# facebookresearch/actionmesh

Hardware: AMD Instinct MI355X
Metric: denoise-steps/sec (16f x 4096tok) (higher is better)
Workload: dtype bf16; 1 GPU; headline: Stage-I denoise step, B=2 (CFG) x T=16 frames x N=4096 tokens, width 1024 (8 heads x 128), 21 layers all inflated, S=257 ctx tokens, random-init weights, seeded N(0,1) latents/context resident in HBM; parallelism=single GPU

## Files before the change

### actionmesh_amd/_lib.py

```python
from __future__ import annotations

import ctypes as C
import os
from typing import Optional

_HERE = os.path.dirname(os.path.abspath(__file__))
LIB_PATH = os.environ.get("ACTIONMESH_AMD_LIB") or os.path.join(_HERE, "libactionmesh_amd.so")
LIB_PATH_F16 = os.environ.get("ACTIONMESH_AMD_LIB_F16") or os.path.join(_HERE, "libactionmesh_amd_f16.so")
ABI_VERSION = 2


class HipLibraryMissing(RuntimeError):
    pass


class AmConfig(C.Structure):
    _fields_ = [
        ("in_channels", C.c_int32), ("num_layers", C.c_int32), ("num_heads", C.c_int32),
        ("width", C.c_int32), ("ff_inner", C.c_int32), ("cross_dim", C.c_int32),
        ("inflated_mask_lo", C.c_uint32), ("inflated_mask_hi", C.c_uint32),
        ("max_batch", C.c_int32), ("max_frames_local", C.c_int32), ("max_tokens", C.c_int32),
        ("max_ctx_tokens", C.c_int32), ("world_size", C.c_int32), ("rank", C.c_int32),
        ("attn_defer_log2", C.c_int32), ("attn_fp8", C.c_int32), ("reserved", C.c_int32 * 6),
    ]


GEMM_ACT_MASK, GEMM_ACT_GELU = 0xff, 1
GEMM_FORCE_128, GEMM_LOCKSTEP, GEMM_FORCE_256 = 0x100, 0x200, 0x400
GEMM_ABLATE_STORE, GEMM_ABLATE_READ, GEMM_ABLATE_MASK = 0x800, 0x1000, 0x1800
GEMM_SKEW_SHIFT, GEMM_SKEW_MASK = 13, 0xe000
GEMM_NO_GELU_TABLE = 0x10000


class AmGemmArgs(C.Structure):
    _fields_ = [
        ("A1", C.c_void_p), ("lda1", C.c_int32), ("K1", C.c_int32),
        ("A2", C.c_void_p), ("lda2", C.c_int32),
        ("W", C.c_void_p), ("ldw", C.c_int32),
        ("bias", C.c_void_p), ("residual", C.c_void_p),
        ("C", C.c_void_p), ("ldc", C.c_int32),
        ("M", C.c_int32), ("N", C.c_int32), ("K", C.c_int32), ("act", C.c_int32),
        ("a_G", C.c_int32), ("a_gs", C.c_int32), ("a_off", C.c_int32),
        ("c_G", C.c_int32), ("c_gs", C.c_int32), ("c_off", C.c_int32),
        ("ln_stats", C.c_void_p), ("ln_colsum", C.c_void_p), ("ln_part", C.c_void_p),
    ]


class AmHeadPostArgs(C.Structure):
    _fields_ = [
        ("X", C.c_void_p), ("ldx", C.c_int32),
        ("rows", C.c_int64), ("seq_len", C.c_int32), ("rows_per_frame", C.c_int32),
        ("heads", C.c_int32), ("nparts", C.c_int32), ("kinds", C.c_int32 * 3),
        ("w_q", C.c_void_p), ("w_k", C.c_void_p), ("eps", C.c_float),
        ("rope_cos", C.c_void_p), ("rope_sin", C.c_void_p),
        ("out_q", C.c_void_p), ("sq_pad", C.c_int32),
        ("out_k", C.c_void_p), ("out_vt", C.c_void_p), ("sk_pad", C.c_int32),
    ]


class AmNnArgs(C.Structure):
    _fields_ = [
        ("points", C.c_void_p), ("n_points", C.c_int64), ("points_bstride", C.c_int64),
        ("queries", C.c_void_p), ("n_queries", C.c_int64), ("queries_bstride", C.c_int64),
        ("batch", C.c_int32), ("precise", C.c_int32),
# ... 316 lines not shown
    "am_image_resample_workspace_bytes": (C.c_size_t, [C.c_int, C.c_int, C.c_int]),
    "am_image_resample": (C.c_int, [C.POINTER(AmImageResampleArgs), _P]),
    "am_image_materialize": (C.c_int, [C.POINTER(AmImageMaterializeArgs), _P]),
    "am_mask_refine_workspace_bytes": (C.c_size_t, [C.c_int, C.c_int, C.c_int]),
    "am_mask_refine": (C.c_int, [C.POINTER(AmMaskRefineArgs), _P]),
    "am_graph_components_workspace_bytes": (C.c_size_t, [C.c_int64, C.c_int64]),
    "am_graph_components": (C.c_int, [C.POINTER(AmGraphArgs), _P]),
    "am_vertex_normals_workspace_bytes": (C.c_size_t, [C.c_int, C.c_int64]),
    "am_vertex_normals": (C.c_int, [C.POINTER(AmVertexNormalsArgs), _P]),
    "am_face_areas": (C.c_int, [C.POINTER(AmFaceAreasArgs), _P]),
    "am_surface_sample": (C.c_int, [C.POINTER(AmSurfaceSampleArgs), _P]),
    "am_decimate_quadrics": (C.c_int, [C.POINTER(AmDecimateQuadricsArgs), _P]),
    "am_decimate_edges": (C.c_int, [C.POINTER(AmDecimateEdgesArgs), _P]),
    "am_decimate_select": (C.c_int, [C.POINTER(AmDecimateSelectArgs), _P]),
    "am_decimate_apply": (C.c_int, [C.POINTER(AmDecimateApplyArgs), _P]),
    "am_iso_classify": (C.c_int, [C.POINTER(AmIsoClassifyArgs), _P]),
    "am_iso_vertices": (C.c_int, [C.POINTER(AmIsoVerticesArgs), _P]),
    "am_iso_triangles": (C.c_int, [C.POINTER(AmIsoTrianglesArgs), _P]),
    "am_dmc_cells": (C.c_int, [C.POINTER(AmDmcCellsArgs), _P]),
    "am_dmc_classify": (C.c_int, [C.POINTER(AmDmcClassifyArgs), _P]),
    "am_dmc_vertices": (C.c_int, [C.POINTER(AmDmcVerticesArgs), _P]),
    "am_dmc_triangles": (C.c_int, [C.POINTER(AmDmcTrianglesArgs), _P]),
    "am_layer_pre_attn": (C.c_int, [_P, C.c_int, _P]),
    "am_layer_attn_local": (C.c_int, [_P, C.c_int, _P]),
    "am_layer_post_attn": (C.c_int, [_P, C.c_int, _P]),
    "am_forward_end": (C.c_int, [_P, _P, _P]),
    "am_kv_chunk_elems": (C.c_int, [_P, C.POINTER(C.c_size_t)]),
    "am_bind_kv_buffers": (C.c_int, [_P, _P, _P, C.c_size_t]),
    "am_bind_kv8_buffers": (C.c_int, [_P, _P, _P, C.c_size_t]),
    "am_attention_counters": (C.c_int, [_P, _P]),
    "am_flow_step": (C.c_int, [_P, _P, C.c_int, _P, C.c_float, C.c_int, _P, C.c_int, C.c_int, C.c_int, _P]),
    "am_step_flops": (C.c_double, [_P, C.c_int, C.c_int, C.c_int, C.c_int]),
    "am_gemm_bf16": (C.c_int, [C.POINTER(AmGemmArgs), _P]),
    "am_layernorm_bf16": (C.c_int, [_P, _P, _P, _P, C.c_int64, C.c_int, C.c_float, _P]),
    "am_add_layernorm_f32": (C.c_int, [_P, _P, _P, _P, _P, C.c_int64, C.c_int, C.c_float, _P]),
    "am_row_stats_bf16": (C.c_int, [_P, _P, C.c_int64, C.c_int, C.c_float, _P]),
    "am_row_stats_finalize": (C.c_int, [_P, C.c_int, C.c_int, _P, C.c_int64, C.c_float, _P]),
    "am_layernorm_stats_bf16": (C.c_int, [_P, _P, _P, _P, C.c_int64, C.c_int, C.c_float, _P, _P]),
    "am_ln_fold_weight": (C.c_int, [_P, _P, _P, _P, _P, _P, _P, C.c_int, C.c_int, _P]),
    "am_head_post": (C.c_int, [C.POINTER(AmHeadPostArgs), _P]),
    "am_gemm_headpost_bf16": (C.c_int, [C.POINTER(AmGemmArgs), C.POINTER(AmHeadPostArgs), _P]),
    "am_attention_bf16": (C.c_int, [C.POINTER(AmAttnArgs), _P]),
    "am_attention_quantize_fp8": (C.c_int, [C.POINTER(AmAttnArgs), _P, _P, _P, _P]),
    "am_attention_fp8": (C.c_int, [C.POINTER(AmAttnArgs), _P, _P, _P, _P]),
    "am_peer_alloc": (C.c_int, [C.c_size_t, C.POINTER(_P)]),
    "am_peer_alloc_flags": (C.c_int, [C.c_size_t, C.POINTER(_P), C.POINTER(C.c_int)]),
    "am_peer_free": (C.c_int, [_P]),
    "am_peer_export": (C.c_int, [_P, _P]),
    "am_peer_open": (C.c_int, [_P, C.POINTER(_P)]),
    "am_peer_close": (C.c_int, [_P]),
    "am_peer_copy": (C.c_int, [_P, _P, C.c_size_t, _P]),
    "am_peer_signal": (C.c_int, [_P, C.c_uint32, _P]),
    "am_peer_wait": (C.c_int, [_P, C.c_uint32, _P, _P]),
    "am_debug_trace_begin": (C.c_int, [_P, C.c_int]),
    "am_debug_trace_end": (C.c_int, [_P, C.c_int, C.POINTER(C.c_int)]),
    "am_debug_trace_stage_name": (C.c_char_p, [C.c_int]),
    "am_f32_to_bf16": (C.c_int, [_P, _P, C.c_size_t, _P]),
    "am_bf16_to_f32": (C.c_int, [_P, _P, C.c_size_t, _P]),
    "am_timestep_sinusoid": (C.c_int, [_P, _P, C.c_int, C.c_int, _P]),
    "am_forward_sharded_peer": (C.c_int, [_P, _P, _P, C.c_int, C.c_int, C.c_int, _P, C.POINTER(AmPeerRing), _P, C.c_int, _P]),
    "am_peer_ring_destroy": (C.c_int, [C.POINTER(AmPeerRing)]),
}

_libs = {}


# ... 52 lines not shown
```

### actionmesh_amd/csrc/am_gemm.hip

```cpp
#include <stdlib.h>
#include <string.h>

#include "am_common.h"

namespace {

constexpr int BM = 128, BN = 128, BK = 64;
constexpr int LDS_ROW = BK + 8;
constexpr int TILE_ELEMS = BM * LDS_ROW;
constexpr int CS_LD = BN + 4;
constexpr int SMEM_MAIN = 2 * 2 * TILE_ELEMS * (int)sizeof(bf16_t);
constexpr int SMEM_EPI = BM * CS_LD * (int)sizeof(float);
constexpr int SMEM_BYTES = SMEM_MAIN > SMEM_EPI ? SMEM_MAIN : SMEM_EPI;
constexpr int GROUP_M = 8;
constexpr int B2 = 256;

__device__ inline int64_t map_row(int r, int G, int gs, int off) {
  if (G <= 0) return r;
  int g = r / G;
  return (int64_t)g * gs + off + (r - g * G);
}

__global__ __launch_bounds__(256, 2) void gemm_bf16_kernel(am_gemm_args p, int tiles_m, int tiles_n, int m_base) {
  extern __shared__ __attribute__((aligned(16))) unsigned char smem[];
  bf16_t* As = reinterpret_cast<bf16_t*>(smem);
  bf16_t* Bs = As + 2 * TILE_ELEMS;
  float* Cs = reinterpret_cast<float*>(smem);

  const int nb = tiles_m * tiles_n;
  const int bid = blockIdx.x;
  int lid;
  {
    const int xcd = bid & 7, idx = bid >> 3;
    const int q = nb >> 3, r = nb & 7;
    lid = (xcd < r ? xcd * (q + 1) : r * (q + 1) + (xcd - r) * q) + idx;
  }
  int tm, tn;
  {
    const int group_sz = GROUP_M * tiles_n;
    const int g = lid / group_sz;
    const int first_m = g * GROUP_M;
    const int gm = min(GROUP_M, tiles_m - first_m);
    const int in_g = lid - g * group_sz;
    tm = first_m + in_g % gm;
    tn = in_g / gm;
  }
  const int m0 = m_base + tm * BM, n0 = tn * BN;
// ... 642 lines not shown
constexpr int GT_ENTRIES = 2 * (int)GT_SPAN;
constexpr int GT_BYTES = GT_ENTRIES * 2;
__global__ void gelu_table_kernel(uint16_t* tab) {
  const int i = blockIdx.x * blockDim.x + threadIdx.x;
  if (i >= GT_ENTRIES) return;
  const uint32_t sgn = (uint32_t)i / GT_SPAN, rel = (uint32_t)i - sgn * GT_SPAN;
  const bf16_t b = (bf16_t)((sgn << 15) | (rel + GT_LO));
  tab[i] = (uint16_t)(pack_bf2(gelu_erf(bf2f(b)), 0.f) & 0xffffu);
}
__device__ __forceinline__ uint32_t gelu_table_pair(uint32_t pk, const unsigned char* tab, uint32_t& bad) {
  const uint32_t b0 = pk & 0xffffu, b1 = pk >> 16;
  const uint32_t r0 = (b0 & 0x7fffu) - GT_LO, r1 = (b1 & 0x7fffu) - GT_LO;
  bad |= (uint32_t)(r0 >= GT_SPAN) | (uint32_t)(r1 >= GT_SPAN);
  const uint32_t i0 = min(r0, GT_SPAN - 1) + (b0 >> 15) * GT_SPAN, i1 = min(r1, GT_SPAN - 1) + (b1 >> 15) * GT_SPAN;
  const uint32_t g0 = *reinterpret_cast<const uint16_t*>(tab + 2u * i0);
  const uint32_t g1 = *reinterpret_cast<const uint16_t*>(tab + 2u * i1);
  return g0 | (g1 << 16);
}
__device__ __forceinline__ bool gelu_table_has(float x) {
  const uint32_t b = pack_bf2(x, 0.f) & 0x7fffu;
  return b - GT_LO < GT_SPAN;
}

constexpr int HT_BYTES = 128 * BK * 2;
constexpr int PBUF_BYTES = 4 * HT_BYTES;
constexpr int FOLD_OFF = 2 * PBUF_BYTES;
constexpr int SMEM2PP_BYTES = FOLD_OFF + 4096;
constexpr int GT_OFF = SMEM2PP_BYTES;
constexpr int SMEM2PP_GELU_BYTES = GT_OFF + GT_BYTES;

#define PP_BARRIER() do { __builtin_amdgcn_sched_barrier(0); asm volatile("s_barrier" ::: "memory"); __builtin_amdgcn_sched_barrier(0); } while (0)
#define PP_LGKM0() asm volatile("s_waitcnt lgkmcnt(0)" ::: "memory")

template <bool HP>
__global__ __launch_bounds__(512, 2) void gemm256pp_bf16_kernel(am_gemm_args p, int tiles_m, int tiles_n, int m_base, am_headpost_args hp,
                                                                 const uint16_t* gelu_tab) {
  extern __shared__ __attribute__((aligned(16))) unsigned char smem[];

  const int nb = tiles_m * tiles_n;
  const int bid = blockIdx.x;
  {
    const int units = (p.act & AM_GEMM_SKEW_MASK) >> AM_GEMM_SKEW_SHIFT;
    if (units && units < 7 && bid < 256) {
      const unsigned long long t0 = wall_clock64();
      const unsigned long long wait = (unsigned long long)(bid & 7) * units * 150ull;
      while (wall_clock64() - t0 < wait) __builtin_amdgcn_s_sleep(4);
    }
  }
  int lid;
  {
    const int xcd = bid & 7, idx = bid >> 3;
    const int q = nb >> 3, r = nb & 7;
    lid = (xcd < r ? xcd * (q + 1) : r * (q + 1) + (xcd - r) * q) + idx;
  }
  int tm, tn;
  {
    const int group_sz = GROUP_M * tiles_n;
    const int g = lid / group_sz;
    const int first_m = g * GROUP_M;
    const int gm = min(GROUP_M, tiles_m - first_m);
    const int in_g = lid - g * group_sz;
    tm = first_m + in_g % gm;
    tn = in_g / gm;
  }
  const int m0 = m_base + tm * B2, n0 = tn * B2;

  const int tid = threadIdx.x;
  const int lane = tid & 63;
  const int wave = __builtin_amdgcn_readfirstlane(tid >> 6);
  const int wm = wave >> 2, wn = wave & 3;

  const int l15 = lane & 15, l4 = lane >> 4;
  f32x4_t acc[8][4];
  {
    f32x4_t bv[4];
#pragma unroll
    for (int ni = 0; ni < 4; ++ni) {
      bv[ni] = f32x4_t{0.f, 0.f, 0.f, 0.f};
      if (p.bias && !p.ln_stats) bv[ni] = *reinterpret_cast<const f32x4_t*>(p.bias + min(n0 + wn * 64 + ni * 16 + l4 * 4, p.N - 4));
    }
#pragma unroll
    for (int ni = 0; ni < 4; ++ni) asm volatile("" : "+v"(bv[ni]));
#pragma unroll
    for (int ni = 0; ni < 4; ++ni)
#pragma unroll
      for (int mi = 0; mi < 8; ++mi) acc[mi][ni] = bv[ni];
  }
  __builtin_amdgcn_sched_barrier(0);
  if (p.ln_stats) {
    {
      const int dw = wave * 64 + lane;
      const int row = min(m0 + (dw >> 1), p.M - 1);
      __builtin_amdgcn_global_load_lds((gbl_ptr_t)(p.ln_stats + 2 * (int64_t)row + (dw & 1)), (lds_ptr_t)(smem + FOLD_OFF + wave * 256), 4, 0, 0);
    }
    {
      const int idx = (wave & 3) * 64 + lane;
      const int n = min(n0 + idx, p.N - 1);
      const float* src = wave < 4 ? p.ln_colsum + n : (p.bias ? p.bias + n : p.ln_colsum + n);
      __builtin_amdgcn_global_load_lds((gbl_ptr_t)src, (lds_ptr_t)(smem + FOLD_OFF + 2048 + wave * 256), 4, 0, 0);
    }
  }

  if (gelu_tab != nullptr) {
#pragma unroll
    for (int i = 0; i < GT_BYTES / 4 / 512; ++i)
      __builtin_amdgcn_global_load_lds((gbl_ptr_t)(reinterpret_cast<const uint32_t*>(gelu_tab) + i * 512 + wave * 64 + lane),
                                       (lds_ptr_t)(smem + GT_OFF + (i * 512 + wave * 64) * 4), 4, 0, 0);
  }

  uint32_t offA1[4], offA2[4], offW[4];
#pragma unroll
  for (int i = 0; i < 4; ++i) {
    const int half = i >> 1, pc = i & 1;
    const int r = pc * 64 + wave * 8 + (lane >> 3);
    const int c = (lane & 7) ^ ((r >> 1) & 7);
    const int ar = min(m0 + half * 128 + r, p.M - 1);
    const int64_t pr = map_row(ar, p.a_G, p.a_gs, p.a_off);
    offA1[i] = (uint32_t)(pr * (p.lda1 >> 3) + c);
    offA2[i] = (uint32_t)(pr * (p.lda2 >> 3) + c);
    const int wr = min(n0 + half * 128 + r, p.N - 1);
    offW[i] = (uint32_t)((int64_t)wr * (p.ldw >> 3) + c);
  }
  auto stage_a = [&](int half, int kt, int buf_off) __attribute__((always_inline)) {
    const int k0 = kt * BK;
    const bool first = k0 < p.K1;
    const unsigned char* base = reinterpret_cast<const unsigned char*>(first ? p.A1 + k0 : p.A2 + (k0 - p.K1));
#pragma unroll
    for (int pc = 0; pc < 2; ++pc) {
      const uint32_t off = first ? offA1[half * 2 + pc] : offA2[half * 2 + pc];
      __builtin_amdgcn_global_load_lds((gbl_ptr_t)(base + ((uint64_t)off << 4)),
                                       (lds_ptr_t)(smem + buf_off + half * HT_BYTES + (pc * 512 + wave * 64) * 16), 16, 0, 0);
    }
  };
  auto stage_w = [&](int half, int kt, int buf_off) __attribute__((always_inline)) {
    const unsigned char* base = reinterpret_cast<const unsigned char*>(p.W + kt * BK);
#pragma unroll
// ... 46 lines not shown
  PP_BARRIER();
  if (wm == 1) PP_BARRIER();

  for (int t = 0; t < nk; ++t) {
    const int cur = (t & 1) * PBUF_BYTES, nxt = PBUF_BYTES - cur;
    const int ta = min(t + 1, nk - 1), tb = min(t + 2, nk - 1);
    read_a(cur, 0); read_w(cur, 0);
    stage_a(0, ta, nxt);
    PP_LGKM0(); PP_BARRIER();
    PP_QUADRANT(0, 0);
    PP_BARRIER();
    read_w(cur, 1);
    stage_a(1, ta, nxt);
    PP_LGKM0(); PP_BARRIER();
    PP_QUADRANT(0, 1);
    PP_BARRIER();
    read_a(cur, 1);
    stage_w(0, tb, cur);
    PP_LGKM0(); PP_BARRIER();
    PP_QUADRANT(1, 1);
    PP_BARRIER();
    stage_w(1, tb, cur);
    asm volatile("s_waitcnt vmcnt(4)" ::: "memory");
    PP_BARRIER();
    PP_QUADRANT(1, 0);
    PP_BARRIER();
  }
  if (wm == 0) PP_BARRIER();
  asm volatile("s_waitcnt vmcnt(0)" ::: "memory");
  PP_BARRIER();

  ResidualPrefetch pre;
  pre.on = false;
  if constexpr (!HP) residual_prefetch(p, tid, m0, n0, pre);
  if (p.ln_stats) {
    f32x4_t cs[4], dv[4];
    const float* fold = reinterpret_cast<const float*>(smem + FOLD_OFF);
#pragma unroll
    for (int ni = 0; ni < 4; ++ni) {
      const int nl = wn * 64 + ni * 16 + l4 * 4;
      cs[ni] = *reinterpret_cast<const f32x4_t*>(fold + 512 + nl);
      dv[ni] = p.bias ? *reinterpret_cast<const f32x4_t*>(fold + 768 + nl) : f32x4_t{0.f, 0.f, 0.f, 0.f};
    }
#pragma unroll
    for (int mi = 0; mi < 8; ++mi) {
      const f32x2_t st = *reinterpret_cast<const f32x2_t*>(fold + 2 * (wm * 128 + mi * 16 + l15));
      const float nm = -st[0] * st[1];
#pragma unroll
      for (int ni = 0; ni < 4; ++ni)
#pragma unroll
        for (int e = 0; e < 4; ++e) acc[mi][ni][e] = fmaf(acc[mi][ni][e], st[1], fmaf(nm, cs[ni][e], dv[ni][e]));
    }
  }
  unsigned char* stage = smem;
  uint32_t gelu_bad = 0;
  auto stage_pass = [&](auto&& convert) __attribute__((always_inline)) {
#pragma unroll
    for (int mi = 0; mi < 8; ++mi)
#pragma unroll
      for (int ni = 0; ni < 4; ++ni) {
        const int ml = wm * 128 + mi * 16 + l15;
        const int nl = wn * 64 + ni * 16 + l4 * 4;
        const u32x2_t w = convert(acc[mi][ni]);
        const int u = (nl >> 2) ^ (ml & 15);
        *reinterpret_cast<u32x2_t*>(stage + ml * 512 + u * 8) = w;
      }
// ... 3 lines not shown
      return u32x2_t{gelu_table_pair(pack_bf2(a[0], a[1]), smem + GT_OFF, gelu_bad), gelu_table_pair(pack_bf2(a[2], a[3]), smem + GT_OFF, gelu_bad)};
    });
  } else if ((p.act & AM_GEMM_ACT_MASK) == AM_GEMM_ACT_GELU) {
    stage_pass([&](const f32x4_t& a) __attribute__((always_inline)) {
      float v[4];
#pragma unroll
      for (int e = 0; e < 4; ++e) v[e] = gelu_erf(rbf(a[e]));
      return u32x2_t{pack_bf2(v[0], v[1]), pack_bf2(v[2], v[3])};
    });
  } else {
    stage_pass([&](const f32x4_t& a) __attribute__((always_inline)) { return u32x2_t{pack_bf2(a[0], a[1]), pack_bf2(a[2], a[3])}; });
  }
  if (gelu_bad) {
#pragma unroll
    for (int mi = 0; mi < 8; ++mi)
#pragma unroll
      for (int ni = 0; ni < 4; ++ni) {
        const int ml = wm * 128 + mi * 16 + l15;
        const int nl = wn * 64 + ni * 16 + l4 * 4;
        bool any = false;
#pragma unroll
        for (int e = 0; e < 4; ++e) any |= !gelu_table_has(acc[mi][ni][e]);
        if (any) {
          uint16_t* q = reinterpret_cast<uint16_t*>(stage + ml * 512 + ((nl >> 2) ^ (ml & 15)) * 8);
#pragma unroll
          for (int e = 0; e < 4; ++e)
            if (!gelu_table_has(acc[mi][ni][e])) q[e] = (uint16_t)(pack_bf2(gelu_erf(rbf(acc[mi][ni][e])), 0.f) & 0xffffu);
        }
      }
  }
  __syncthreads();
  if constexpr (HP) store_staged_tile_headpost(p, hp, stage, tid, m0, n0);
  else store_staged_tile(p, stage, tid, m0, n0, &pre);
}
#undef PP_QUADRANT

}

static int gemm_skew_units(int rounds) {
  static int enabled[64];
  int dev = 0;
  if (hipGetDevice(&dev) != hipSuccess || dev < 0 || dev >= 64) return 0;
  if (enabled[dev] == 0) {
    hipDeviceProp_t pr;
    bool on = hipGetDeviceProperties(&pr, dev) == hipSuccess && pr.multiProcessorCount == 256 && strncmp(pr.gcnArchName, "gfx950", 6) == 0;
    const char* e = getenv("ACTIONMESH_AMD_GEMM_SKEW");
    if (e && e[0] == '0') on = false;
    enabled[dev] = on ? 1 : 2;
  }
  if (enabled[dev] != 1) return 0;
  return rounds >= 24 ? 4 : rounds >= 16 ? 3 : rounds >= 12 ? 2 : rounds >= 4 ? 1 : 0;
}

static const uint16_t* gelu_table(hipStream_t st) {
#ifdef AM_F16
  return nullptr;
#else
  static uint16_t* tab[64];
  static int state[64];
  static std::mutex mu;
  int dev = 0, cur = 0;
  if (hipGetDevice(&cur) != hipSuccess) return nullptr;
  dev = cur;
  if (st != nullptr && hipStreamGetDevice(st, &dev) != hipSuccess) { (void)hipGetLastError(); dev = cur; }
  if (dev < 0 || dev >= 64) return nullptr;
  std::lock_guard<std::mutex> lk(mu);
  if (state[dev] == 0) {
    const char* e = getenv("ACTIONMESH_AMD_GELU_TABLE");
    if (e && e[0] == '0') { state[dev] = 2; return nullptr; }
    hipStreamCaptureStatus cs = hipStreamCaptureStatusNone;
    if (hipStreamIsCapturing(st, &cs) != hipSuccess || cs != hipStreamCaptureStatusNone) { (void)hipGetLastError(); return nullptr; }
    if (dev != cur && hipSetDevice(dev) != hipSuccess) { (void)hipGetLastError(); return nullptr; }
    uint16_t* t = nullptr;
    bool ok = hipMalloc(reinterpret_cast<void**>(&t), GT_BYTES) == hipSuccess;
    if (ok) {
      hipLaunchKernelGGL(gelu_table_kernel, dim3(ceil_div(GT_ENTRIES, 256)), dim3(256), 0, st, t);
      ok = hipGetLastError() == hipSuccess && hipStreamSynchronize(st) == hipSuccess;
      if (!ok) (void)hipFree(t);
    }
    if (dev != cur) (void)hipSetDevice(cur);
    if (!ok) { (void)hipGetLastError(); return nullptr; }
    tab[dev] = t;
    state[dev] = 1;
  }
// ... 15 lines not shown
  }
}

extern "C" int am_gemm_bf16(const am_gemm_args* a, void* stream) {
  AM_CHECK(a != nullptr, "am_gemm_bf16: null args");
  AM_CHECK(a->M > 0 && a->N > 0 && a->K > 0, "am_gemm_bf16: empty problem M=%d N=%d K=%d", a->M, a->N, a->K);
  AM_CHECK(a->K % BK == 0, "am_gemm_bf16: K=%d must be a multiple of %d", a->K, BK);
  AM_CHECK(a->N % 8 == 0, "am_gemm_bf16: N=%d must be a multiple of 8", a->N);
  AM_CHECK(a->A1 && a->W && a->C, "am_gemm_bf16: null operand");
  AM_CHECK(a->K1 > 0 && a->K1 <= a->K && a->K1 % BK == 0, "am_gemm_bf16: K1=%d invalid for K=%d", a->K1, a->K);
  AM_CHECK(a->K1 == a->K || a->A2 != nullptr, "am_gemm_bf16: K1 < K requires A2");
  AM_CHECK(a->lda1 % 8 == 0 && a->ldw % 8 == 0 && a->ldc % 8 == 0 && (a->A2 == nullptr || a->lda2 % 8 == 0),
           "am_gemm_bf16: leading dimensions must be multiples of 8 elements (16 B)");
  AM_CHECK(((uintptr_t)a->A1 | (uintptr_t)a->W | (uintptr_t)a->C | (uintptr_t)a->A2 | (uintptr_t)a->residual) % 16 == 0,
           "am_gemm_bf16: operands must be 16-byte aligned");
  if (a->ln_stats) {
    AM_CHECK(a->ln_colsum != nullptr, "am_gemm_bf16: ln_stats without ln_colsum");
    AM_CHECK(a->A2 == nullptr, "am_gemm_bf16: a folded LayerNorm needs one A operand");
    AM_CHECK(a->a_G == 0 || (a->act & AM_GEMM_FORCE_128) || (a->N < 256 && !(a->act & AM_GEMM_FORCE_256)),
             "am_gemm_bf16: a folded LayerNorm over a row-mapped A needs the 128x128 kernel (N < 256 without the forced 256x256 tile)");
    AM_CHECK(!(a->act & AM_GEMM_LOCKSTEP), "am_gemm_bf16: the round-1 lockstep kernel has no folded-LayerNorm epilogue");
    AM_CHECK(((uintptr_t)a->ln_stats % 8 == 0) && ((uintptr_t)a->ln_colsum % 16 == 0) && (a->bias == nullptr || (uintptr_t)a->bias % 16 == 0) &&
             a->N % 4 == 0, "am_gemm_bf16: ln_stats / ln_colsum / bias misaligned");
  }
  if (a->ln_part) {
    AM_CHECK(a->c_G == 0, "am_gemm_bf16: ln_part needs the identity C row map");
    AM_CHECK((uintptr_t)a->ln_part % 8 == 0, "am_gemm_bf16: ln_part misaligned");
  }
  AM_ONCE_PER_DEVICE({
    AM_HIP(hipFuncSetAttribute(reinterpret_cast<const void*>(gemm_bf16_kernel),
                               hipFuncAttributeMaxDynamicSharedMemorySize, SMEM_BYTES));
    AM_HIP(hipFuncSetAttribute(reinterpret_cast<const void*>(gemm256_bf16_kernel),
                               hipFuncAttributeMaxDynamicSharedMemorySize, SMEM2_BYTES));
    AM_HIP(hipFuncSetAttribute(reinterpret_cast<const void*>(gemm256pp_bf16_kernel<false>),
                               hipFuncAttributeMaxDynamicSharedMemorySize, SMEM2PP_GELU_BYTES));
    AM_HIP(hipFuncSetAttribute(reinterpret_cast<const void*>(gemm256pp_bf16_kernel<true>),
                               hipFuncAttributeMaxDynamicSharedMemorySize, SMEM2PP_BYTES));
  });
  am_gemm_args args = *a;
  const bool force_small = (args.act & AM_GEMM_FORCE_128) != 0;
  const bool legacy = (args.act & AM_GEMM_LOCKSTEP) != 0;
  const bool force_big = (args.act & AM_GEMM_FORCE_256) != 0;
  const int abl = args.act & (AM_GEMM_ABLATE_MASK | AM_GEMM_SKEW_MASK);
  const bool no_gelu_table = (args.act & AM_GEMM_NO_GELU_TABLE) != 0;
  args.act &= AM_GEMM_ACT_MASK;
  AM_CHECK(args.act == 0 || args.act == AM_GEMM_ACT_GELU, "am_gemm_bf16: unknown activation %d", args.act);
  const bool big = !force_small && args.N >= 8 && args.M >= 1 &&
                   (force_big || (args.N >= 256 && args.M >= 1024 && (int64_t)ceil_div(args.M, B2) * ceil_div(args.N, B2) >= 192));
  AM_CHECK(!big || (uintptr_t)args.bias % 16 == 0, "am_gemm_bf16: the 256x256 tile needs a 16-byte aligned bias");
  args.act |= abl;
  float* const ln_part = args.ln_part;
  int64_t part_done = 0;
  args.ln_part = nullptr;
  if (big && (abl & AM_GEMM_SKEW_MASK) == 0) {
    const int rounds = (int)(((int64_t)ceil_div(args.M, B2) * ceil_div(args.N, B2)) / 256);
    args.act |= gemm_skew_units(rounds) << AM_GEMM_SKEW_SHIFT;
  }
  if (big) {
    const int rem = args.M % B2;
    const int m_main = (rem != 0 && rem <= 128 && args.M > 8 * B2) ? args.M - rem : args.M;
    const int tiles_m = ceil_div(m_main, B2), tiles_n = ceil_div(args.N, B2);
    if (legacy) {
      hipLaunchKernelGGL(gemm256_bf16_kernel, dim3(tiles_m * tiles_n), dim3(512), SMEM2_BYTES,
                         (hipStream_t)stream, args, tiles_m, tiles_n, 0);
    } else {
      am_gemm_args main_args = args;
      if (ln_part && args.N % B2 == 0 && !(args.act & AM_GEMM_ABLATE_MASK)) {
        main_args.ln_part = ln_part;
        part_done = (int64_t)(args.M / B2) * B2;
        if (part_done > m_main) part_done = m_main;
      }
      const uint16_t* gt = ((main_args.act & AM_GEMM_ACT_MASK) == AM_GEMM_ACT_GELU && !no_gelu_table) ? gelu_table((hipStream_t)stream) : nullptr;
      hipLaunchKernelGGL(gemm256pp_bf16_kernel<false>, dim3(tiles_m * tiles_n), dim3(512), gt ? SMEM2PP_GELU_BYTES : SMEM2PP_BYTES,
                         (hipStream_t)stream, main_args, tiles_m, tiles_n, 0, am_headpost_args{}, gt);
    }
    if (m_main < args.M) launch_tail(args, m_main, (hipStream_t)stream);
  } else {
    const int tiles_m = ceil_div(args.M, BM), tiles_n = ceil_div(args.N, BN);
    hipLaunchKernelGGL(gemm_bf16_kernel, dim3(tiles_m * tiles_n), dim3(256), SMEM_BYTES,
                       (hipStream_t)stream, args, tiles_m, tiles_n, 0);
  }
  AM_HIP(hipGetLastError());
  if (ln_part && part_done < args.M)
    AM_TRY(am_row_part(args.C, args.ldc, part_done, args.M - part_done, args.N, ln_part, stream));
  return AM_OK;
}

int am_head_post_partial(const am_headpost_args* a, int s_min_last, int s_min_other, void* stream);

extern "C" int am_gemm_headpost_bf16(const am_gemm_args* g, const am_headpost_args* hp, void* stream) {
  AM_CHECK(g && hp, "am_gemm_headpost_bf16: null argument");
  AM_CHECK(g->C == hp->X && g->ldc == hp->ldx && (int64_t)g->M == hp->rows && g->N == hp->heads * hp->nparts * 128,
           "am_gemm_headpost_bf16: the GEMM's output (C, ldc, M, N) must be the head split's input (X, ldx, rows, heads * nparts * 128)");
  bool has_v = false;
  for (int i = 0; i < hp->nparts; ++i) has_v |= hp->kinds[i] == 2;
  const int rem = g->M % B2;
  const bool tail_split = rem != 0 && rem <= 128 && g->M > 8 * B2;
  AM_CHECK(g->ln_part == nullptr, "am_gemm_headpost_bf16: no row statistics of a head-split output");
  const bool fuse = (g->act & AM_GEMM_ACT_MASK) == 0 && !g->residual && (!g->bias || g->ln_stats) && !g->A2 && g->a_G == 0 && g->c_G == 0 && g->N % 256 == 0 && g->M % 16 == 0 &&
                    g->N >= 256 && g->M >= 1024 && (int64_t)ceil_div(g->M, B2) * ceil_div(g->N, B2) >= 192 &&
                    (!has_v || hp->seq_len % 16 == 0) && (!tail_split || rem <= hp->seq_len) && hp->rows % hp->seq_len == 0 &&
                    !(g->act & (AM_GEMM_FORCE_128 | AM_GEMM_LOCKSTEP | AM_GEMM_FORCE_256)) && getenv("ACTIONMESH_AMD_NO_FUSED_QKV") == nullptr;
  if (!fuse) {
    AM_TRY(am_gemm_bf16(g, stream));
    return am_head_post(hp, stream);
  }
  AM_CHECK(g->K % BK == 0 && g->K1 == g->K && g->lda1 % 8 == 0 && g->ldw % 8 == 0, "am_gemm_headpost_bf16: bad GEMM operands");
  AM_CHECK(((uintptr_t)g->A1 | (uintptr_t)g->W | (uintptr_t)g->C) % 16 == 0, "am_gemm_headpost_bf16: operands must be 16-byte aligned");
  if (g->ln_stats)
    AM_CHECK(g->ln_colsum && (uintptr_t)g->ln_stats % 8 == 0 && (uintptr_t)g->ln_colsum % 16 == 0 && (g->bias == nullptr || (uintptr_t)g->bias % 16 == 0),
             "am_gemm_headpost_bf16: ln_stats / ln_colsum / bias missing or misaligned");
  AM_TRY(am_head_post_check(hp));
  AM_ONCE_PER_DEVICE({
    AM_HIP(hipFuncSetAttribute(reinterpret_cast<const void*>(gemm256pp_bf16_kernel<true>), hipFuncAttributeMaxDynamicSharedMemorySize, SMEM2PP_BYTES));
    AM_HIP(hipFuncSetAttribute(reinterpret_cast<const void*>(gemm_bf16_kernel), hipFuncAttributeMaxDynamicSharedMemorySize, SMEM_BYTES));
  });
  am_gemm_args args = *g;
  args.act = g->act & AM_GEMM_ABLATE_MASK;
  const int m_main = tail_split ? args.M - rem : args.M;
  const int tiles_m = ceil_div(m_main, B2), tiles_n = ceil_div(args.N, B2);
  {
    const int rounds = (int)(((int64_t)tiles_m * tiles_n) / 256);
    args.act |= gemm_skew_units(rounds) << AM_GEMM_SKEW_SHIFT;
  }
  am_gemm_args main_args = args;
  main_args.M = m_main;
  hipLaunchKernelGGL(gemm256pp_bf16_kernel<true>, dim3(tiles_m * tiles_n), dim3(512), SMEM2PP_BYTES, (hipStream_t)stream, main_args, tiles_m,
                     tiles_n, 0, *hp, (const uint16_t*)nullptr);
  if (m_main < args.M) launch_tail(args, m_main, (hipStream_t)stream);
  AM_HIP(hipGetLastError());
  const int s_min_last = hp->seq_len - (args.M - m_main);
  return am_head_post_partial(hp, s_min_last, hp->seq_len, stream);
}
```

### actionmesh_amd/ops.py

```python
from __future__ import annotations

import ctypes as C
from typing import Optional, Sequence, Tuple

import torch

from . import _lib as L
from .mesh_topology import MeshTopology

HEAD_DIM = 128


H16 = (torch.bfloat16, torch.float16)


def _entry(key, name: str):
    if isinstance(key, torch.Tensor):
        key = key.dtype
    l = L.lib(key if isinstance(key, str) else "f16" if key == torch.float16 else "bf16")
    return l, getattr(l, name)


def _call(t: torch.Tensor, key, name: str, *args) -> None:
    l, fn = _entry(key, name)
# ... 26 lines not shown


def _need_rows(t: torch.Tensor, dtype, name: str) -> torch.Tensor:
    _on_device(t, dtype, name)
    if t.dim() != 2 or t.stride(1) != 1:
        raise ValueError(f"{name}: expected a 2-D tensor with unit column stride, got shape {tuple(t.shape)} strides {t.stride()}")
    return t


def round_up(x: int, m: int) -> int:
    return (x + m - 1) // m * m


def _out_rows(out: Optional[torch.Tensor], rows: int, ld_out: int, dtype, device, name: str) -> torch.Tensor:
    if out is None:
        return torch.empty((rows, ld_out), dtype=dtype, device=device)
    _need(out, dtype, f"{name}: out")
    if tuple(out.shape) != (rows, ld_out):
        raise ValueError(f"{name}: out {tuple(out.shape)} != ({rows}, {ld_out})")
    return out


def perm16_index(n: int, device=None) -> torch.Tensor:
    k = torch.arange(n, device=device)
    return (k & ~0xC) | ((k & 4) << 1) | ((k & 8) >> 1)


def _fold_args(g, bias: Optional[torch.Tensor], ln: Optional[Tuple[torch.Tensor, torch.Tensor]]) -> None:
    if bias is not None:
        g.bias = _need(bias, torch.float32, "bias").data_ptr()
    if ln is not None:
        g.ln_stats = _need(ln[0], torch.float32, "ln stats").data_ptr()
        g.ln_colsum = _need(ln[1], torch.float32, "ln colsum").data_ptr()


def gemm(a: torch.Tensor, w: torch.Tensor, bias: Optional[torch.Tensor] = None,
         residual: Optional[torch.Tensor] = None, gelu: bool = False,
         a2: Optional[torch.Tensor] = None, out: Optional[torch.Tensor] = None,
         a_map: Tuple[int, int, int] = (0, 0, 0), c_map: Tuple[int, int, int] = (0, 0, 0),
         M: Optional[int] = None, force_small: bool = False, legacy: bool = False,
         force_big: bool = False, ablate: int = 0,
         ln: Optional[Tuple[torch.Tensor, torch.Tensor]] = None, ln_part: Optional[torch.Tensor] = None,
         gelu_table: bool = True) -> torch.Tensor:
    _need_rows(a, H16, "a"); _need_rows(w, a.dtype, "w")
    K1 = a.shape[1]
    K = w.shape[1]
    N = w.shape[0]
    if M is None:
        M = a.shape[0]
    if out is None:
        out = torch.empty((M, N), dtype=a.dtype, device=a.device)
    _need_rows(out, a.dtype, "out")
    g = L.AmGemmArgs()
    g.A1 = a.data_ptr(); g.lda1 = a.stride(0); g.K1 = K1
    g.A2 = _p(a2); g.lda2 = a2.stride(0) if a2 is not None else 0
    if a2 is not None:
        _need_rows(a2, a.dtype, "a2")
        assert K1 + a2.shape[1] == K
    else:
        assert K1 == K
    g.W = w.data_ptr(); g.ldw = w.stride(0)
    _fold_args(g, bias, ln)
    g.residual = _p(_need_rows(residual, a.dtype, "residual")) if residual is not None else None
    g.C = out.data_ptr(); g.ldc = out.stride(0)
    g.M, g.N, g.K = M, N, K
    g.act = (L.GEMM_ACT_GELU if gelu else 0) | (L.GEMM_FORCE_128 if force_small else 0) | (L.GEMM_LOCKSTEP if legacy else 0) \
        | (L.GEMM_FORCE_256 if force_big else 0) | (ablate & (L.GEMM_ABLATE_MASK | L.GEMM_SKEW_MASK)) | (0 if gelu_table else L.GEMM_NO_GELU_TABLE)
    g.a_G, g.a_gs, g.a_off = a_map
    g.c_G, g.c_gs, g.c_off = c_map
    if ln is not None:
        assert ln[0].numel() >= 2 * M and ln[1].numel() == N
    if ln_part is not None:
        _need(ln_part, torch.float32, "ln_part")
        assert ln_part.numel() >= 2 * M * ((N + 255) // 256)
        g.ln_part = ln_part.data_ptr()
    _call(a, a, "am_gemm_bf16", C.byref(g))
    return out


def row_stats(x: torch.Tensor, eps: float = 1e-5, out: Optional[torch.Tensor] = None) -> torch.Tensor:
    _need(x, H16, "x")
    Cdim = x.shape[-1]
    rows = x.numel() // Cdim
    if out is None:
        out = torch.empty((rows, 2), dtype=torch.float32, device=x.device)
    _call(x, x, "am_row_stats_bf16", x.data_ptr(), _need(out, torch.float32, "out").data_ptr(), rows, Cdim, eps)
    return out


def row_stats_finalize(part: torch.Tensor, Cdim: int, eps: float = 1e-5, out: Optional[torch.Tensor] = None, kind=torch.bfloat16) -> torch.Tensor:
    _need(part, torch.float32, "part")
    rows, nparts = part.shape[0], part.shape[1]
    if out is None:
        out = torch.empty((rows, 2), dtype=torch.float32, device=part.device)
    _call(part, kind, "am_row_stats_finalize", part.data_ptr(), nparts, Cdim, out.data_ptr(), rows, eps)
    return out


def ln_fold_weight(w: torch.Tensor, gamma: torch.Tensor, beta: torch.Tensor, bias: Optional[torch.Tensor] = None,
                   out: Optional[Tuple[torch.Tensor, torch.Tensor, torch.Tensor]] = None):
# ... 77 lines not shown
    h.sk_pad = out_k.shape[2] if out_k is not None else (out_vt.shape[3] if out_vt is not None else 0)
    return h, (out_q, out_k, out_vt)


def head_post(x: torch.Tensor, heads: int, kinds: Sequence[int], seq_len: int, rows_per_frame: int,
              w_q: Optional[torch.Tensor] = None, w_k: Optional[torch.Tensor] = None,
              rope: Optional[Tuple[torch.Tensor, torch.Tensor]] = None, eps: float = 1e-6,
              out_q: Optional[torch.Tensor] = None, out_k: Optional[torch.Tensor] = None,
              out_vt: Optional[torch.Tensor] = None):
    _need_rows(x, H16, "x")
    h, outs = _head_post_args(x, heads, kinds, seq_len, rows_per_frame, w_q, w_k, rope, eps, out_q, out_k, out_vt)
    _call(x, x, "am_head_post", C.byref(h))
    return outs


def gemm_head_post(a: torch.Tensor, w: torch.Tensor, heads: int, kinds: Sequence[int], seq_len: int, rows_per_frame: int,
                   w_q: Optional[torch.Tensor] = None, w_k: Optional[torch.Tensor] = None,
                   rope: Optional[Tuple[torch.Tensor, torch.Tensor]] = None, eps: float = 1e-6,
                   out_q: Optional[torch.Tensor] = None, out_k: Optional[torch.Tensor] = None,
                   out_vt: Optional[torch.Tensor] = None, x: Optional[torch.Tensor] = None,
                   bias: Optional[torch.Tensor] = None, ln: Optional[Tuple[torch.Tensor, torch.Tensor]] = None, ablate: int = 0):
    _need(a, H16, "a"); _need(w, a.dtype, "w")
    rows, K = a.shape
    N = w.shape[0]
    assert N == heads * len(kinds) * HEAD_DIM and w.shape[1] == K
    if x is None:
        x = torch.empty((rows, N), dtype=a.dtype, device=a.device)
    _need_rows(x, a.dtype, "x")
    g = L.AmGemmArgs()
    g.A1 = a.data_ptr(); g.lda1 = a.stride(0); g.K1 = K
    g.W = w.data_ptr(); g.ldw = w.stride(0)
    g.C = x.data_ptr(); g.ldc = x.stride(0)
    g.M, g.N, g.K = rows, N, K
    g.act = ablate & L.GEMM_ABLATE_MASK
    _fold_args(g, bias, ln)
    h, outs = _head_post_args(x, heads, kinds, seq_len, rows_per_frame, w_q, w_k, rope, eps, out_q, out_k, out_vt)
    _call(a, a, "am_gemm_headpost_bf16", C.byref(g), C.byref(h))
    return outs


STATE_LD = 132


def _attn_args(q: torch.Tensor, k: torch.Tensor, vt: torch.Tensor, sq: int, sk: int, out: Optional[torch.Tensor], nchunks: int,
               scale: Optional[float], defer_log2: int, rows: int, state_mode: int, state: Optional[torch.Tensor], chunk_first: int,
               chunk_total: int):
    _need(q, H16, "q"); _need(k, q.dtype, "k"); _need(vt, q.dtype, "vt")
    nseq, H, sq_pad, _ = q.shape
    sk_pad = k.shape[-2]
    if out is None:
        out = torch.empty((nseq * sq, H * HEAD_DIM), dtype=q.dtype, device=q.device)
    _need_rows(out, q.dtype, "out")
    a = L.AmAttnArgs()
    a.Q, a.K, a.Vt, a.O = q.data_ptr(), k.data_ptr(), vt.data_ptr(), out.data_ptr()
    a.nseq, a.heads, a.sq, a.sq_pad, a.sk, a.sk_pad = nseq, H, sq, sq_pad, sk, sk_pad
    a.nchunks = nchunks
    a.chunk_stride = nseq * H * sk_pad * HEAD_DIM
    a.ldo = out.stride(0)
    a.scale = scale if scale is not None else HEAD_DIM ** -0.5
    a.defer_log2 = defer_log2
    a.rows, a.state_mode, a.chunk_first, a.chunk_total = rows, state_mode, chunk_first, chunk_total
    if state is not None:
        _need(state, torch.float32, "state")
        assert state.numel() >= nseq * H * sq_pad * STATE_LD
        a.state = state.data_ptr()
    return a, out

# ... 1028 lines not shown
```

### include/actionmesh_amd.h

```cpp
#ifndef ACTIONMESH_AMD_H
#define ACTIONMESH_AMD_H

#include <stddef.h>
#include <stdint.h>

#ifdef __cplusplus
extern "C" {
#endif

typedef enum {
  AM_OK = 0,
  AM_ERR_INVALID = -1,
  AM_ERR_HIP = -2,
  AM_ERR_STATE = -3,
  AM_ERR_NOTFOUND = -4
} am_status;

const char* am_last_error(void);
int am_abi_version(void);


typedef struct {
  int32_t in_channels;
  int32_t num_layers;
// ... 44 lines not shown
int am_kv_chunk_elems(am_handle h, size_t* elems_per_chunk);
int am_bind_kv_buffers(am_handle h, uint16_t* k_dev, uint16_t* vt_dev, size_t chunk_stride_elems);

int am_bind_kv8_buffers(am_handle h, uint8_t* k8_dev, uint8_t* vt8_dev, size_t chunk_stride_bytes);
int am_attention_counters(am_handle h, uint64_t* counts2);

int am_flow_step(const uint16_t* v_dev, float* latents_dev, int n_branches,
                 const float* scales_host, float dt, int is_additive,
                 const uint8_t* unobserved_host, int T_local, int N, int Din, void* stream);

double am_step_flops(am_handle h, int B, int T_total, int N, int S);


typedef struct {
  const uint16_t* A1; int32_t lda1; int32_t K1;
  const uint16_t* A2; int32_t lda2;
  const uint16_t* W;  int32_t ldw;
  const float* bias;
  const uint16_t* residual;
  uint16_t* C; int32_t ldc;
  int32_t M, N, K;
  int32_t act;
#define AM_GEMM_ACT_MASK      0xff
#define AM_GEMM_ACT_GELU      1
#define AM_GEMM_FORCE_128     0x100
#define AM_GEMM_LOCKSTEP      0x200
#define AM_GEMM_FORCE_256     0x400
#define AM_GEMM_ABLATE_STORE  0x800
#define AM_GEMM_ABLATE_READ   0x1000
#define AM_GEMM_ABLATE_MASK   0x1800
#define AM_GEMM_SKEW_SHIFT    13
#define AM_GEMM_SKEW_MASK     0xe000
#define AM_GEMM_NO_GELU_TABLE 0x10000
  int32_t a_G, a_gs, a_off;
  int32_t c_G, c_gs, c_off;
  const float* ln_stats;
  const float* ln_colsum;
  float* ln_part;
} am_gemm_args;
int am_gemm_bf16(const am_gemm_args* args, void* stream);

int am_row_stats_bf16(const uint16_t* x, float* stats, int64_t rows, int C, float eps, void* stream);
int am_row_stats_finalize(const float* part, int nparts, int C, float* stats, int64_t rows, float eps, void* stream);
int am_layernorm_stats_bf16(const uint16_t* x, uint16_t* y, const float* w, const float* b,
                            int64_t rows, int C, float eps, float* stats_y, void* stream);
int am_ln_fold_weight(const uint16_t* W, const float* gamma, const float* beta, const float* bias, uint16_t* Wf, float* colsum,
                      float* d, int N, int K, void* stream);

int am_layernorm_bf16(const uint16_t* x, uint16_t* y, const float* w, const float* b,
                      int64_t rows, int C, float eps, void* stream);

int am_add_layernorm_f32(float* h32, const uint16_t* y16, uint16_t* z16, const float* w, const float* b, int64_t rows, int C, float eps,
                         void* stream);

typedef struct {
  const uint16_t* X; int32_t ldx;
  int64_t rows; int32_t seq_len; int32_t rows_per_frame;
  int32_t heads; int32_t nparts; int32_t kinds[3];
  const float* w_q; const float* w_k; float eps;
  const float* rope_cos; const float* rope_sin;
  uint16_t* out_q; int32_t sq_pad;
  uint16_t* out_k; uint16_t* out_vt; int32_t sk_pad;
} am_headpost_args;
int am_head_post(const am_headpost_args* args, void* stream);

int am_gemm_headpost_bf16(const am_gemm_args* gemm, const am_headpost_args* headpost, void* stream);

typedef struct {
  const uint16_t* Q; const uint16_t* K; const uint16_t* Vt; uint16_t* O;
  int32_t nseq, heads, sq, sq_pad, sk, sk_pad, nchunks;
  int64_t chunk_stride;
  int32_t ldo; float scale; int32_t defer_log2;
  int32_t chunk_first, chunk_total, rows, state_mode;
// ... 489 lines not shown
```

Measured before the change: 1.508 denoise-steps/s.

## Make ping-pong 256 GEMM persistent with CU-sized grid and tile loop

Measured after the change: 1.506 denoise-steps/s. Within noise of the previous version (-0.1%).

```diff
diff --git a/actionmesh_amd/_lib.py b/actionmesh_amd/_lib.py
--- a/actionmesh_amd/_lib.py
+++ b/actionmesh_amd/_lib.py
@@ -30,6 +30,8 @@
 GEMM_ABLATE_STORE, GEMM_ABLATE_READ, GEMM_ABLATE_MASK = 0x800, 0x1000, 0x1800
 GEMM_SKEW_SHIFT, GEMM_SKEW_MASK = 13, 0xe000
 GEMM_NO_GELU_TABLE = 0x10000
+GEMM_ONE_TILE = 0x20000
+GEMM_RESIDENT_SHIFT, GEMM_RESIDENT_MASK = 18, 0x3c0000
 
 
 class AmGemmArgs(C.Structure):
@@ -412,6 +414,7 @@
     "am_flow_step": (C.c_int, [_P, _P, C.c_int, _P, C.c_float, C.c_int, _P, C.c_int, C.c_int, C.c_int, _P]),
     "am_step_flops": (C.c_double, [_P, C.c_int, C.c_int, C.c_int, C.c_int]),
     "am_gemm_bf16": (C.c_int, [C.POINTER(AmGemmArgs), _P]),
+    "am_gemm_tile_walk": (C.c_int, [C.c_int, C.c_int, C.c_int, C.c_int, C.c_int, C.POINTER(C.c_int), C.POINTER(C.c_int)]),
     "am_layernorm_bf16": (C.c_int, [_P, _P, _P, _P, C.c_int64, C.c_int, C.c_float, _P]),
     "am_add_layernorm_f32": (C.c_int, [_P, _P, _P, _P, _P, C.c_int64, C.c_int, C.c_float, _P]),
     "am_row_stats_bf16": (C.c_int, [_P, _P, C.c_int64, C.c_int, C.c_float, _P]),
diff --git a/actionmesh_amd/csrc/am_gemm.hip b/actionmesh_amd/csrc/am_gemm.hip
--- a/actionmesh_amd/csrc/am_gemm.hip
+++ b/actionmesh_amd/csrc/am_gemm.hip
@@ -2,6 +2,7 @@
 #include <string.h>
 
 #include "am_common.h"
+#include "am_gemm_walk.h"
 
 namespace {
 
@@ -12,7 +13,6 @@
 constexpr int SMEM_MAIN = 2 * 2 * TILE_ELEMS * (int)sizeof(bf16_t);
 constexpr int SMEM_EPI = BM * CS_LD * (int)sizeof(float);
 constexpr int SMEM_BYTES = SMEM_MAIN > SMEM_EPI ? SMEM_MAIN : SMEM_EPI;
-constexpr int GROUP_M = 8;
 constexpr int B2 = 256;
 
 __device__ inline int64_t map_row(int r, int G, int gs, int off) {
@@ -721,43 +721,58 @@
 #define PP_BARRIER() do { __builtin_amdgcn_sched_barrier(0); asm volatile("s_barrier" ::: "memory"); __builtin_amdgcn_sched_barrier(0); } while (0)
 #define PP_LGKM0() asm volatile("s_waitcnt lgkmcnt(0)" ::: "memory")
 
-template <bool HP>
-__global__ __launch_bounds__(512, 2) void gemm256pp_bf16_kernel(am_gemm_args p, int tiles_m, int tiles_n, int m_base, am_headpost_args hp,
+struct gemm256pp_kernargs {
+  am_gemm_args p; int tiles_m, tiles_n, m_base; am_headpost_args hp; const uint16_t* gelu_tab;
+};
+#define AM_ASSUME_GLOBAL(PTR) do { auto g_ = (__attribute__((address_space(1))) void*)(void*)(PTR); asm volatile("" : "+s"(g_)); PTR = (decltype(PTR))g_; } while (0)
+typedef const __attribute__((address_space(4))) uint32_t* kernarg_words_t;
+template <typename T>
+__device__ __forceinline__ T load_kernarg(kernarg_words_t src) {
+  static_assert(sizeof(T) % 4 == 0 && alignof(T) <= 8, "kernel arguments are read as dwords");
+  struct Words { uint32_t w[sizeof(T) / 4]; } t;
+#pragma unroll
+  for (size_t i = 0; i < sizeof(T) / 4; ++i) t.w[i] = src[i];
+  return __builtin_bit_cast(T, t);
+}
+template <bool HP, bool RES>
+__global__ __launch_bounds__(512, 2) void gemm256pp_bf16_kernel(am_gemm_args p_in, int tiles_m, int tiles_n, int m_base, am_headpost_args hp_in,
                                                                  const uint16_t* gelu_tab) {
   extern __shared__ __attribute__((aligned(16))) unsigned char smem[];
 
   const int nb = tiles_m * tiles_n;
   const int bid = blockIdx.x;
+  if (RES && bid >= nb) return;
   {
-    const int units = (p.act & AM_GEMM_SKEW_MASK) >> AM_GEMM_SKEW_SHIFT;
+    const int units = (p_in.act & AM_GEMM_SKEW_MASK) >> AM_GEMM_SKEW_SHIFT;
     if (units && units < 7 && bid < 256) {
       const unsigned long long t0 = wall_clock64();
       const unsigned long long wait = (unsigned long long)(bid & 7) * units * 150ull;
       while (wall_clock64() - t0 < wait) __builtin_amdgcn_s_sleep(4);
     }
   }
-  int lid;
-  {
-    const int xcd = bid & 7, idx = bid >> 3;
-    const int q = nb >> 3, r = nb & 7;
-    lid = (xcd < r ? xcd * (q + 1) : r * (q + 1) + (xcd - r) * q) + idx;
-  }
-  int tm, tn;
-  {
-    const int group_sz = GROUP_M * tiles_n;
-    const int g = lid / group_sz;
-    const int first_m = g * GROUP_M;
-    const int gm = min(GROUP_M, tiles_m - first_m);
-    const int in_g = lid - g * group_sz;
-    tm = first_m + in_g % gm;
-    tn = in_g / gm;
-  }
-  const int m0 = m_base + tm * B2, n0 = tn * B2;
-
-  const int tid = threadIdx.x;
+  int v = bid;
+  do {
+  int tid = threadIdx.x;
+  am_gemm_args p;
+  am_headpost_args hp;
+  if constexpr (RES) {
+    asm volatile("" : "+v"(tid));
+    kernarg_words_t ka = (kernarg_words_t)__builtin_amdgcn_kernarg_segment_ptr();
+    asm volatile("" : "+s"(ka));
+    p = load_kernarg<am_gemm_args>(ka + offsetof(gemm256pp_kernargs, p) / 4);
+    AM_ASSUME_GLOBAL(p.A1); AM_ASSUME_GLOBAL(p.A2); AM_ASSUME_GLOBAL(p.W); AM_ASSUME_GLOBAL(p.bias); AM_ASSUME_GLOBAL(p.residual);
+    AM_ASSUME_GLOBAL(p.C); AM_ASSUME_GLOBAL(p.ln_stats); AM_ASSUME_GLOBAL(p.ln_colsum); AM_ASSUME_GLOBAL(p.ln_part);
+    hp = hp_in;
+  } else {
+    p = p_in;
+    hp = hp_in;
+  }
   const int lane = tid & 63;
   const int wave = __builtin_amdgcn_readfirstlane(tid >> 6);
   const int wm = wave >> 2, wn = wave & 3;
+  int tm, tn;
+  gemm_tile_of_block(v, tiles_m, tiles_n, tm, tn);
+  const int m0 = m_base + tm * B2, n0 = tn * B2;
 
   const int l15 = lane & 15, l4 = lane >> 4;
   f32x4_t acc[8][4];
@@ -790,7 +805,7 @@
     }
   }
 
-  if (gelu_tab != nullptr) {
+  if (gelu_tab != nullptr && v == bid) {
 #pragma unroll
     for (int i = 0; i < GT_BYTES / 4 / 512; ++i)
       __builtin_amdgcn_global_load_lds((gbl_ptr_t)(reinterpret_cast<const uint32_t*>(gelu_tab) + i * 512 + wave * 64 + lane),
@@ -903,6 +918,10 @@
 
   ResidualPrefetch pre;
   pre.on = false;
+  if constexpr (RES) {
+#pragma unroll
+    for (int i = 0; i < 16; ++i) pre.rv[i] = u32x4_t{0u, 0u, 0u, 0u};
+  }
   if constexpr (!HP) residual_prefetch(p, tid, m0, n0, pre);
   if (p.ln_stats) {
     f32x4_t cs[4], dv[4];
@@ -972,6 +991,11 @@
   __syncthreads();
   if constexpr (HP) store_staged_tile_headpost(p, hp, stage, tid, m0, n0);
   else store_staged_tile(p, stage, tid, m0, n0, &pre);
+  if constexpr (!RES) break;
+  v += gridDim.x;
+  if (v >= nb) break;
+  __syncthreads();
+  } while (true);
 }
 #undef PP_QUADRANT
 
@@ -990,6 +1014,42 @@
   }
   if (enabled[dev] != 1) return 0;
   return rounds >= 24 ? 4 : rounds >= 16 ? 3 : rounds >= 12 ? 2 : rounds >= 4 ? 1 : 0;
+}
+
+static int gemm_resident_grid(int64_t tiles, int act) {
+  static int units[64];
+  if (act & AM_GEMM_ONE_TILE) return 0;
+  int dev = 0;
+  if (hipGetDevice(&dev) != hipSuccess || dev < 0 || dev >= 64) return 0;
+  if (units[dev] == 0) {
+    hipDeviceProp_t pr;
+    int n = hipGetDeviceProperties(&pr, dev) == hipSuccess ? pr.multiProcessorCount : 0;
+    const char* e = getenv("ACTIONMESH_AMD_GEMM_RESIDENT");
+    if (e && e[0] == '0') n = 0;
+    units[dev] = n > 0 ? n : -1;
+  }
+  if (units[dev] < 0) return 0;
+  const int cap = units[dev] > 8 ? units[dev] & ~7 : units[dev];
+  const int f = (act & AM_GEMM_RESIDENT_MASK) >> AM_GEMM_RESIDENT_SHIFT;
+  if (f) return 8 * f < cap ? 8 * f : cap;
+  const int g = tiles < cap ? (int)tiles : cap;
+  return g > 8 ? g & ~7 : g;
+}
+
+template <bool HP>
+static void launch_pingpong(int act_switches, size_t smem, hipStream_t st, const am_gemm_args& a, int tiles_m, int tiles_n,
+                            const am_headpost_args& hp, const uint16_t* gt) {
+  const int64_t tiles = (int64_t)tiles_m * tiles_n;
+  const int G = gemm_resident_grid(tiles, act_switches);
+  if (G > 0) hipLaunchKernelGGL((gemm256pp_bf16_kernel<HP, true>), dim3(G), dim3(512), smem, st, a, tiles_m, tiles_n, 0, hp, gt);
+  else hipLaunchKernelGGL((gemm256pp_bf16_kernel<HP, false>), dim3((unsigned)tiles), dim3(512), smem, st, a, tiles_m, tiles_n, 0, hp, gt);
+}
+
+extern "C" int am_gemm_tile_walk(int tiles_m, int tiles_n, int G, int block, int trip, int* tm, int* tn) {
+  int m = 0, n = 0;
+  if (tm == nullptr || tn == nullptr || !gemm_tile_walk(tiles_m, tiles_n, G, block, trip, m, n)) return 0;
+  *tm = m; *tn = n;
+  return 1;
 }
 
 static const uint16_t* gelu_table(hipStream_t st) {
@@ -1071,9 +1131,13 @@
                                hipFuncAttributeMaxDynamicSharedMemorySize, SMEM_BYTES));
     AM_HIP(hipFuncSetAttribute(reinterpret_cast<const void*>(gemm256_bf16_kernel),
                                hipFuncAttributeMaxDynamicSharedMemorySize, SMEM2_BYTES));
-    AM_HIP(hipFuncSetAttribute(reinterpret_cast<const void*>(gemm256pp_bf16_kernel<false>),
+    AM_HIP(hipFuncSetAttribute(reinterpret_cast<const void*>(gemm256pp_bf16_kernel<false, false>),
                                hipFuncAttributeMaxDynamicSharedMemorySize, SMEM2PP_GELU_BYTES));
-    AM_HIP(hipFuncSetAttribute(reinterpret_cast<const void*>(gemm256pp_bf16_kernel<true>),
+    AM_HIP(hipFuncSetAttribute(reinterpret_cast<const void*>(gemm256pp_bf16_kernel<false, true>),
+                               hipFuncAttributeMaxDynamicSharedMemorySize, SMEM2PP_GELU_BYTES));
+    AM_HIP(hipFuncSetAttribute(reinterpret_cast<const void*>(gemm256pp_bf16_kernel<true, false>),
+                               hipFuncAttributeMaxDynamicSharedMemorySize, SMEM2PP_BYTES));
+    AM_HIP(hipFuncSetAttribute(reinterpret_cast<const void*>(gemm256pp_bf16_kernel<true, true>),
                                hipFuncAttributeMaxDynamicSharedMemorySize, SMEM2PP_BYTES));
   });
   am_gemm_args args = *a;
@@ -1082,6 +1146,7 @@
   const bool force_big = (args.act & AM_GEMM_FORCE_256) != 0;
   const int abl = args.act & (AM_GEMM_ABLATE_MASK | AM_GEMM_SKEW_MASK);
   const bool no_gelu_table = (args.act & AM_GEMM_NO_GELU_TABLE) != 0;
+  const int resident = args.act & (AM_GEMM_ONE_TILE | AM_GEMM_RESIDENT_MASK);
   args.act &= AM_GEMM_ACT_MASK;
   AM_CHECK(args.act == 0 || args.act == AM_GEMM_ACT_GELU, "am_gemm_bf16: unknown activation %d", args.act);
   const bool big = !force_small && args.N >= 8 && args.M >= 1 &&
@@ -1110,8 +1175,8 @@
         if (part_done > m_main) part_done = m_main;
       }
       const uint16_t* gt = ((main_args.act & AM_GEMM_ACT_MASK) == AM_GEMM_ACT_GELU && !no_gelu_table) ? gelu_table((hipStream_t)stream) : nullptr;
-      hipLaunchKernelGGL(gemm256pp_bf16_kernel<false>, dim3(tiles_m * tiles_n), dim3(512), gt ? SMEM2PP_GELU_BYTES : SMEM2PP_BYTES,
-                         (hipStream_t)stream, main_args, tiles_m, tiles_n, 0, am_headpost_args{}, gt);
+      launch_pingpong<false>(resident, gt ? SMEM2PP_GELU_BYTES : SMEM2PP_BYTES, (hipStream_t)stream, main_args, tiles_m, tiles_n,
+                             am_headpost_args{}, gt);
     }
     if (m_main < args.M) launch_tail(args, m_main, (hipStream_t)stream);
   } else {
@@ -1151,7 +1216,8 @@
              "am_gemm_headpost_bf16: ln_stats / ln_colsum / bias missing or misaligned");
   AM_TRY(am_head_post_check(hp));
   AM_ONCE_PER_DEVICE({
-    AM_HIP(hipFuncSetAttribute(reinterpret_cast<const void*>(gemm256pp_bf16_kernel<true>), hipFuncAttributeMaxDynamicSharedMemorySize, SMEM2PP_BYTES));
+    AM_HIP(hipFuncSetAttribute(reinterpret_cast<const void*>(gemm256pp_bf16_kernel<true, false>), hipFuncAttributeMaxDynamicSharedMemorySize, SMEM2PP_BYTES));
+    AM_HIP(hipFuncSetAttribute(reinterpret_cast<const void*>(gemm256pp_bf16_kernel<true, true>), hipFuncAttributeMaxDynamicSharedMemorySize, SMEM2PP_BYTES));
     AM_HIP(hipFuncSetAttribute(reinterpret_cast<const void*>(gemm_bf16_kernel), hipFuncAttributeMaxDynamicSharedMemorySize, SMEM_BYTES));
   });
   am_gemm_args args = *g;
@@ -1164,8 +1230,8 @@
   }
   am_gemm_args main_args = args;
   main_args.M = m_main;
-  hipLaunchKernelGGL(gemm256pp_bf16_kernel<true>, dim3(tiles_m * tiles_n), dim3(512), SMEM2PP_BYTES, (hipStream_t)stream, main_args, tiles_m,
-                     tiles_n, 0, *hp, (const uint16_t*)nullptr);
+  launch_pingpong<true>(g->act & (AM_GEMM_ONE_TILE | AM_GEMM_RESIDENT_MASK), SMEM2PP_BYTES, (hipStream_t)stream, main_args, tiles_m, tiles_n, *hp,
+                        (const uint16_t*)nullptr);
   if (m_main < args.M) launch_tail(args, m_main, (hipStream_t)stream);
   AM_HIP(hipGetLastError());
   const int s_min_last = hp->seq_len - (args.M - m_main);
diff --git a/actionmesh_amd/csrc/am_gemm_walk.h b/actionmesh_amd/csrc/am_gemm_walk.h
--- /dev/null
+++ b/actionmesh_amd/csrc/am_gemm_walk.h
@@ -0,0 +1,25 @@
+#pragma once
+
+constexpr int GROUP_M = 8;
+
+__host__ __device__ inline void gemm_tile_of_block(int v, int tiles_m, int tiles_n, int& tm, int& tn) {
+  const int nb = tiles_m * tiles_n;
+  const int xcd = v & 7, idx = v >> 3;
+  const int q = nb >> 3, r = nb & 7;
+  const int lid = (xcd < r ? xcd * (q + 1) : r * (q + 1) + (xcd - r) * q) + idx;
+  const int group_sz = GROUP_M * tiles_n;
+  const int g = lid / group_sz;
+  const int first_m = g * GROUP_M;
+  const int gm = tiles_m - first_m < GROUP_M ? tiles_m - first_m : GROUP_M;
+  const int in_g = lid - g * group_sz;
+  tm = first_m + in_g % gm;
+  tn = in_g / gm;
+}
+
+__host__ __device__ inline bool gemm_tile_walk(int tiles_m, int tiles_n, int G, int block, int trip, int& tm, int& tn) {
+  if (tiles_m <= 0 || tiles_n <= 0 || G <= 0 || block < 0 || block >= G || trip < 0) return false;
+  const long long v = (long long)block + (long long)trip * G;
+  if (v >= (long long)tiles_m * tiles_n) return false;
+  gemm_tile_of_block((int)v, tiles_m, tiles_n, tm, tn);
+  return true;
+}
diff --git a/actionmesh_amd/ops.py b/actionmesh_amd/ops.py
--- a/actionmesh_amd/ops.py
+++ b/actionmesh_amd/ops.py
@@ -82,6 +82,9 @@
     if ln is not None:
         g.ln_stats = _need(ln[0], torch.float32, "ln stats").data_ptr()
         g.ln_colsum = _need(ln[1], torch.float32, "ln colsum").data_ptr()
+
+
+_GEMM_SWITCHES = L.GEMM_ABLATE_MASK | L.GEMM_SKEW_MASK | L.GEMM_ONE_TILE | L.GEMM_RESIDENT_MASK
 
 
 def gemm(a: torch.Tensor, w: torch.Tensor, bias: Optional[torch.Tensor] = None,
@@ -115,7 +118,7 @@
     g.C = out.data_ptr(); g.ldc = out.stride(0)
     g.M, g.N, g.K = M, N, K
     g.act = (L.GEMM_ACT_GELU if gelu else 0) | (L.GEMM_FORCE_128 if force_small else 0) | (L.GEMM_LOCKSTEP if legacy else 0) \
-        | (L.GEMM_FORCE_256 if force_big else 0) | (ablate & (L.GEMM_ABLATE_MASK | L.GEMM_SKEW_MASK)) | (0 if gelu_table else L.GEMM_NO_GELU_TABLE)
+        | (L.GEMM_FORCE_256 if force_big else 0) | (ablate & _GEMM_SWITCHES) | (0 if gelu_table else L.GEMM_NO_GELU_TABLE)
     g.a_G, g.a_gs, g.a_off = a_map
     g.c_G, g.c_gs, g.c_off = c_map
     if ln is not None:
@@ -259,7 +262,7 @@
     g.W = w.data_ptr(); g.ldw = w.stride(0)
     g.C = x.data_ptr(); g.ldc = x.stride(0)
     g.M, g.N, g.K = rows, N, K
-    g.act = ablate & L.GEMM_ABLATE_MASK
+    g.act = ablate & (L.GEMM_ABLATE_MASK | L.GEMM_ONE_TILE | L.GEMM_RESIDENT_MASK)
     _fold_args(g, bias, ln)
     h, outs = _head_post_args(x, heads, kinds, seq_len, rows_per_frame, w_q, w_k, rope, eps, out_q, out_k, out_vt)
     _call(a, a, "am_gemm_headpost_bf16", C.byref(g), C.byref(h))
diff --git a/include/actionmesh_amd.h b/include/actionmesh_amd.h
--- a/include/actionmesh_amd.h
+++ b/include/actionmesh_amd.h
@@ -100,6 +100,9 @@
 #define AM_GEMM_SKEW_SHIFT    13
 #define AM_GEMM_SKEW_MASK     0xe000
 #define AM_GEMM_NO_GELU_TABLE 0x10000
+#define AM_GEMM_ONE_TILE      0x20000
+#define AM_GEMM_RESIDENT_SHIFT 18
+#define AM_GEMM_RESIDENT_MASK 0x3c0000
   int32_t a_G, a_gs, a_off;
   int32_t c_G, c_gs, c_off;
   const float* ln_stats;
@@ -107,6 +110,7 @@
   float* ln_part;
 } am_gemm_args;
 int am_gemm_bf16(const am_gemm_args* args, void* stream);
+int am_gemm_tile_walk(int tiles_m, int tiles_n, int G, int block, int trip, int* tm, int* tn);
 
 int am_row_stats_bf16(const uint16_t* x, float* stats, int64_t rows, int C, float eps, void* stream);
 int am_row_stats_finalize(const float* part, int nparts, int C, float* stats, int64_t rows, float eps, void* stream);
```
